# ZhangXinWhut/SimWhisper-Codec

Hardware: AMD Instinct MI355X
Metric: audio-sec/sec encode+decode (RTF^-1), 16kHz batch=32x10s (higher is better)
Workload: dtype split-f16 x3 encode (f32-class, f32 accumulate) / bf16 decode (f32 accumulate); 1 GPU; batch=32x10s @16kHz per GPU (32 utterances in all), encode()+decode(), 0.1*N(0,1) seed 1234, synthetic closed-form checkpoint (291M params); precision=mixed

## Files before the change

### include/swc.h

```cpp
#ifndef SWC_H_
#define SWC_H_

#include <stdint.h>

#ifdef __cplusplus
extern "C" {
#endif

#define SWC_OK 0
#define SWC_E_ARG (-1)
#define SWC_E_LAUNCH (-2)
#define SWC_E_NODEV (-3)

#define SWC_F32 0
#define SWC_BF16 1
#define SWC_F16S 2
#define SWC_F16S_ACT_SCALE 64.0f
#define SWC_FP8 3
#define SWC_FP8_ACT_SCALE 16.0f
#define SWC_F16 4

#define SWC_ACT_NONE 0
#define SWC_ACT_GELU 1

int swc_version(void);
const char* swc_last_error(void);
int swc_device_count(void);

int swc_delay_us(int32_t us, void* stream);

int swc_set_saturation_counter(uint32_t* counters);

typedef struct swc_gemm_args {
    const void* A;
    const void* W;
    void* C;
    const float* bias;
    const float* gamma;
    const float* residual;
    int64_t lda, ldw, ldc, ldr;
    int32_t M, N, K;
    int32_t taps, dil, stride, pad, t_in, t_out;
    int32_t a_dtype, c_dtype, act;
    float alpha;
    float out_scale;
} swc_gemm_args;
int swc_gemm(const swc_gemm_args* args, void* stream);

int swc_attention(const void* qkv, void* out, const int32_t* lens, int32_t B, int32_t T,
                  int32_t H, int32_t dtype, void* stream);
int swc_attention16(const void* qkv, void* out, const int32_t* lens, int32_t B, int32_t T, int32_t H,
                    int32_t dtype, const int32_t* row_start, void* stream);
int swc_attention_ex(const void* qkv, void* out, const int32_t* lens, int32_t B, int32_t T, int32_t H,
                     int32_t out_dtype, void* stream);

int swc_layernorm(const float* x, void* y, const float* w, const float* b, const int32_t* lens,
                  int32_t B, int32_t t_in, int32_t t_out, int32_t C, float eps, int32_t y_dtype,
                  const int32_t* row_start, void* stream);

int swc_pack_rows(const void* src, void* dst, const int32_t* row_start, const int32_t* lens, int32_t B, int32_t T,
                  int64_t row_bytes, void* stream);

int64_t swc_convnext_stream_bytes(int32_t C, int32_t I);
int swc_convnext_pack(const void* w1_16bit, const void* w2_16bit, const float* gamma, void* w_stream, int32_t C, int32_t I,
                      void* stream);
int swc_convnext_mlp(const void* y, const void* w_stream, const float* b1, const float* b2, const float* gamma,
                     float* x, int32_t M, int32_t C, int32_t I, void* stream);
int swc_convnext_block(const float* x, float* x_out, const float* dw_w7, const float* dw_bias, const float* ln_w,
                       const float* ln_b, float eps, const void* w_stream, const float* b1, const float* b2,
                       const float* gamma, int32_t B, int32_t T, int32_t C, int32_t I, const int32_t* t_limit,
                       int32_t operand_dtype, void* stream);

int64_t swc_convnext64_stream_bytes(int32_t C, int32_t I);
int swc_convnext64_pack(const void* w1_bf16, const void* w2_bf16, void* w_stream, int32_t C, int32_t I, void* stream);
int swc_convnext64_mlp(const void* y, const void* w_stream, const float* b1, const float* b2, const float* gamma, float* x,
                       int32_t M, int32_t C, int32_t I, int32_t stagger_cycles, void* stream);

int64_t swc_mlp_stream_bytes(int32_t D, int32_t F);
int swc_mlp_pack(const void* w1_bf16, const void* w2_bf16, void* w_stream, int32_t D, int32_t F, void* stream);
int swc_mlp_block(const float* x, float* x_out, const float* ln_w, const float* ln_b, float eps, const void* w_stream,
                  const float* b1, const float* b2, const float* next_ln_w, const float* next_ln_b, void* y_next,
                  int32_t M, int32_t D, int32_t F, void* stream);

int64_t swc_layer_tail_stream_bytes(int32_t D, int32_t F, int32_t fc1_dtype);
int swc_layer_tail_pack(const void* wo_bf16, const void* w1, const void* w2_bf16, void* w_stream, int32_t D, int32_t F,
                        int32_t fc1_dtype, void* stream);
int swc_layer_tail(const void* attn, const float* x, float* x_out, const void* w_stream, const float* bo, const float* ln_w,
                   const float* ln_b, float eps, const float* b1, const float* b2, const float* next_ln_w,
                   const float* next_ln_b, void* y_next, int32_t M, int32_t D, int32_t F, int32_t fc1_dtype, float fc1_alpha,
                   int32_t operand_dtype, void* stream);

int64_t swc_proj_ln_stream_bytes(int32_t N, int32_t K);
int swc_proj_ln_pack(const void* w_f16s, void* w_stream, int32_t N, int32_t K, void* stream);
int swc_proj_ln(const void* a_f16s, int64_t lda, const void* w_stream, const float* bias, float alpha, const float* x,
                float* x_out, const float* ln_w, const float* ln_b, float eps, void* y_next, int32_t M, int32_t N, int32_t K,
                void* stream);

int swc_dwconv7_ln(const float* x, void* y, const float* w, const float* bias, const float* ln_w,
                   const float* ln_b, int32_t B, int32_t T, int32_t C, float eps, int32_t y_dtype,
                   void* stream);

int swc_snake_aa(const float* x, void* y, const float* alpha, const float* beta,
                 const float* filt_host12, int32_t B, int32_t T, int32_t C, int32_t y_dtype,
                 void* stream);

int swc_fsq_encode(const float* z, int64_t ldz, float* zq, int32_t* codes, const int32_t* lens,
                   const float* consts_host12, int32_t B, int32_t T, int32_t t_pad, int32_t G,
                   void* stream);
int swc_fsq_decode(const int64_t* codes, float* zq, int64_t ldq, const int32_t* lens, int32_t B,
                   int32_t T, int32_t G, void* stream);
int swc_fsq_encode_levels(const float* z, int64_t ldz, float* zq, int32_t* codes, const int32_t* lens,
                          const float* consts_host12, const int32_t* levels_host4, int32_t B, int32_t T,
                          int32_t t_pad, int32_t G, void* stream);
int swc_fsq_decode_levels(const int64_t* codes, float* zq, int64_t ldq, const int32_t* lens,
                          const int32_t* levels_host4, int32_t B, int32_t T, int32_t G, void* stream);

int swc_mel_frames(const float* wav, int64_t ld_wav, const int32_t* n, int32_t n_pad,
                   float* frames, int32_t B, int32_t T, void* stream);
int swc_mel_power(const float* dft, int64_t ld, float* pw, int64_t ldp, int64_t rows,
                  void* stream);
int swc_mel_logmax(float* mel, int64_t ld, float* umax, int32_t B, int32_t T, int32_t n_mel,
                   void* stream);
int swc_mel_final(const float* mel, int64_t ld, const float* umax, void* out, int64_t ldo,
                  int32_t B, int32_t T, int32_t n_mel, int32_t out_dtype, void* stream);

int swc_deconv_col2im(const float* y3, const float* bias, void* out, int64_t ldo, int32_t B,
                      int32_t T, int32_t C, int32_t s, int32_t t_out, int32_t out_dtype,
                      void* stream);

int swc_istft_spec(const float* h, int64_t ldh, void* s, int64_t lds, int64_t rows,
                   int32_t s_dtype, void* stream);
int swc_istft_ola(const float* frames, const float* window_sq, float* wav, int32_t B, int32_t T,
                  void* stream);

int swc_codes_pack(const int32_t* codes, int64_t ldg, void* bytes, int32_t T, void* stream);
int swc_codes_unpack(const void* bytes, int32_t* codes, int64_t ldg, int32_t T, void* stream);

int swc_cast_f32_bf16(const float* x, void* y, int64_t n, void* stream);
int swc_cast_f32_f16s(const float* x, int64_t ldx, void* y, int64_t rows, int32_t K, float scale,
                      void* stream);
int swc_cast_fp8(const void* x, int32_t x_dtype, void* y, int64_t n, float scale, void* stream);

int swc_gather_rows(const void* const* src, const int64_t* nbytes, void* out, int64_t ld_bytes, int32_t n_rows,
                    void* stream);

int swc_pcm16_to_f32(const int16_t* pcm, float* out, int64_t n, void* stream);
int swc_f32_to_pcm16(const float* x, int16_t* pcm, int64_t n, void* stream);


#ifdef __cplusplus
}
#endif
#endif
```

### simwhisper_codec_amd/_lib.py

```python
import ctypes as C
import os

import torch

HERE = os.path.dirname(os.path.abspath(__file__))
LIB_PATH = os.environ.get("SWC_LIB") or os.path.join(HERE, "libswc_hip.so")

F32, BF16, F16S, FP8 = 0, 1, 2, 3
F16S_ACT_SCALE = 64.0
FP8_ACT_SCALE = 16.0
ACT_NONE, ACT_GELU = 0, 1


class SwcError(RuntimeError):
    pass


class GemmArgs(C.Structure):
    _fields_ = [
        ("A", C.c_void_p), ("W", C.c_void_p), ("C", C.c_void_p),
        ("bias", C.c_void_p), ("gamma", C.c_void_p), ("residual", C.c_void_p),
        ("lda", C.c_int64), ("ldw", C.c_int64), ("ldc", C.c_int64), ("ldr", C.c_int64),
        ("M", C.c_int32), ("N", C.c_int32), ("K", C.c_int32),
        ("taps", C.c_int32), ("dil", C.c_int32), ("stride", C.c_int32), ("pad", C.c_int32),
        ("t_in", C.c_int32), ("t_out", C.c_int32),
        ("a_dtype", C.c_int32), ("c_dtype", C.c_int32), ("act", C.c_int32),
        ("alpha", C.c_float), ("out_scale", C.c_float),
    ]


_P, _I, _L, _F = C.c_void_p, C.c_int32, C.c_int64, C.c_float

SIGNATURES = {
    "swc_gemm": [C.POINTER(GemmArgs), _P],
    "swc_attention": [_P, _P, _P, _I, _I, _I, _I, _P],
    "swc_attention_ex": [_P, _P, _P, _I, _I, _I, _I, _P],
    "swc_attention16": [_P, _P, _P, _I, _I, _I, _I, _P, _P],
    "swc_layernorm": [_P, _P, _P, _P, _P, _I, _I, _I, _I, _F, _I, _P, _P],
    "swc_dwconv7_ln": [_P, _P, _P, _P, _P, _P, _I, _I, _I, _F, _I, _P],
    "swc_snake_aa": [_P, _P, _P, _P, C.POINTER(_F), _I, _I, _I, _I, _P],
    "swc_fsq_encode": [_P, _L, _P, _P, _P, C.POINTER(_F), _I, _I, _I, _I, _P],
    "swc_fsq_decode": [_P, _P, _L, _P, _I, _I, _I, _P],
    "swc_fsq_encode_levels": [_P, _L, _P, _P, _P, C.POINTER(_F), C.POINTER(C.c_int32), _I, _I, _I, _I, _P],
    "swc_fsq_decode_levels": [_P, _P, _L, _P, C.POINTER(C.c_int32), _I, _I, _I, _P],
    "swc_mel_frames": [_P, _L, _P, _I, _P, _I, _I, _P],
    "swc_mel_power": [_P, _L, _P, _L, _L, _P],
    "swc_mel_logmax": [_P, _L, _P, _I, _I, _I, _P],
    "swc_mel_final": [_P, _L, _P, _P, _L, _I, _I, _I, _I, _P],
    "swc_deconv_col2im": [_P, _P, _P, _L, _I, _I, _I, _I, _I, _I, _P],
    "swc_istft_spec": [_P, _L, _P, _L, _L, _I, _P],
    "swc_istft_ola": [_P, _P, _P, _I, _I, _P],
    "swc_codes_pack": [_P, _L, _P, _I, _P],
    "swc_codes_unpack": [_P, _P, _L, _I, _P],
    "swc_cast_f32_bf16": [_P, _P, _L, _P],
    "swc_cast_f32_f16s": [_P, _L, _P, _L, _I, _F, _P],
    "swc_cast_fp8": [_P, _I, _P, _L, _F, _P],
    "swc_gather_rows": [_P, _P, _P, _L, _I, _P],
    "swc_pcm16_to_f32": [_P, _P, _L, _P],
    "swc_f32_to_pcm16": [_P, _P, _L, _P],
    "swc_set_saturation_counter": [_P],
    "swc_delay_us": [_I, _P],
    "swc_pack_rows": [_P, _P, _P, _P, _I, _I, _L, _P],
    "swc_convnext_pack": [_P, _P, _P, _P, _I, _I, _P],
    "swc_convnext_mlp": [_P, _P, _P, _P, _P, _P, _I, _I, _I, _P],
    "swc_convnext_block": [_P, _P, _P, _P, _P, _P, _F, _P, _P, _P, _P, _I, _I, _I, _I, _P, _I, _P],
    "swc_convnext64_pack": [_P, _P, _P, _I, _I, _P],
    "swc_convnext64_mlp": [_P, _P, _P, _P, _P, _P, _I, _I, _I, _I, _P],
    "swc_mlp_pack": [_P, _P, _P, _I, _I, _P],
    "swc_mlp_block": [_P, _P, _P, _P, _F, _P, _P, _P, _P, _P, _P, _I, _I, _I, _P],
    "swc_layer_tail_pack": [_P, _P, _P, _P, _I, _I, _I, _P],
    "swc_layer_tail": [_P, _P, _P, _P, _P, _P, _P, _F, _P, _P, _P, _P, _P, _I, _I, _I, _I, _F, _I, _P],
    "swc_proj_ln_pack": [_P, _P, _I, _I, _P],
    "swc_proj_ln": [_P, _L, _P, _P, _F, _P, _P, _P, _P, _F, _P, _I, _I, _I, _P],
}
PLAIN = {"swc_version": ([], C.c_int), "swc_last_error": ([], C.c_char_p), "swc_device_count": ([], C.c_int),
         "swc_convnext_stream_bytes": ([_I, _I], C.c_int64),
         "swc_mlp_stream_bytes": ([_I, _I], C.c_int64), "swc_convnext64_stream_bytes": ([_I, _I], C.c_int64), "swc_layer_tail_stream_bytes": ([_I, _I, _I], C.c_int64),
         "swc_proj_ln_stream_bytes": ([_I, _I], C.c_int64)}

_lib = None


def load():
    global _lib
    if _lib is not None:
        return _lib
    if not os.path.exists(LIB_PATH):
        raise SwcError(
            f"{LIB_PATH} is missing: build it with `python -m simwhisper_codec_amd.build` "
            "(there is no CPU or PyTorch fallback for the hot path)")
    lib = C.CDLL(LIB_PATH)
    for name, argtypes in SIGNATURES.items():
        fn = getattr(lib, name)
        fn.argtypes = argtypes
        fn.restype = C.c_int
    for name, (argtypes, restype) in PLAIN.items():
        fn = getattr(lib, name)
        fn.argtypes = argtypes
        fn.restype = restype
    _lib = lib
    return lib


def check(rc, what):
    if rc != 0:
        msg = load().swc_last_error().decode("utf-8", "replace")
        raise SwcError(f"{what} failed (rc={rc}): {msg}")


def exported_symbols():
    return list(SIGNATURES) + list(PLAIN)
```

### simwhisper_codec_amd/csrc/swc_attention16.hip

```cpp
#include "swc_common.h"
#include <type_traits>

namespace {

typedef short s16x4 __attribute__((ext_vector_type(4)));
typedef short s16x8 __attribute__((ext_vector_type(8)));

__device__ __attribute__((aligned(16))) unsigned int g_zero16a[4] = {0u, 0u, 0u, 0u};

__device__ __forceinline__ void glds16a(const void* gsrc, unsigned lds_addr) {
    unsigned keep;
    asm volatile(
        "s_mov_b32 %0, m0\n\ts_mov_b32 m0, %2\n\ts_nop 0\n\tglobal_load_lds_dwordx4 %1, off\n\ts_mov_b32 m0, %0"
        : "=&s"(keep)
        : "v"(gsrc), "s"(lds_addr)
        : "memory");
}

typedef unsigned u32x2_sw __attribute__((ext_vector_type(2)));
template <int W>
__device__ __forceinline__ float xor_max(float v) {
    const unsigned u = __float_as_uint(v);
    const u32x2_sw r = W == 16 ? __builtin_amdgcn_permlane16_swap(u, u, false, false) : __builtin_amdgcn_permlane32_swap(u, u, false, false);
    return fmaxf(__uint_as_float(r[0]), __uint_as_float(r[1]));
}

template <int PLANES>
__device__ __forceinline__ f32x4 mma16(const uint4& a, const uint4& b, f32x4 c) {
#if defined(ATT_ABL) && (ATT_ABL & 8)
    c[0] += __uint_as_float(a.x ^ b.x);
    return c;
#endif
    if constexpr (PLANES == 1)
        return __builtin_amdgcn_mfma_f32_16x16x32_bf16(*reinterpret_cast<const bf16x8*>(&a),
                                                       *reinterpret_cast<const bf16x8*>(&b), c, 0, 0, 0);
    else
        return __builtin_amdgcn_mfma_f32_16x16x32_f16(*reinterpret_cast<const f16x8*>(&a),
                                                      *reinterpret_cast<const f16x8*>(&b), c, 0, 0, 0);
}

typedef float f32x2 __attribute__((ext_vector_type(2)));
typedef __bf16 bf16x2n __attribute__((ext_vector_type(2)));
typedef _Float16 f16x2 __attribute__((ext_vector_type(2)));
__device__ __forceinline__ unsigned pack2_bf16(float lo, float hi) {
    const bf16x2n r = __builtin_convertvector((f32x2){lo, hi}, bf16x2n);
    return *reinterpret_cast<const unsigned*>(&r);
}
__device__ __forceinline__ unsigned pack2_f16(float lo, float hi) {
    const f16x2 r = __builtin_convertvector((f32x2){lo, hi}, f16x2);
    return *reinterpret_cast<const unsigned*>(&r);
}


template <int PLANES, int KT16, int NQT, bool RES = false>
__global__ __launch_bounds__(RES ? 512 : 256, RES ? 1 : (NQT == 1 ? 4 : 2)) void attn16_kernel(const char* __restrict__ qkv, unsigned short* __restrict__ out,
                                                        const int* __restrict__ lens, int T, int H,
                                                        const int* __restrict__ row_start) {
    constexpr int ROWB = 128 * PLANES;
    constexpr int CPR = ROWB / 16;
    constexpr int TILE = KT16 * ROWB;
    constexpr int QB16 = 64 * NQT;
    constexpr int QW = 16 * NQT;
    constexpr int NKS = KT16 / 16;
    constexpr int NPR = KT16 / 32;
    constexpr int NI = TILE / 1024;
    extern __shared__ __attribute__((aligned(16))) char smem[];

    constexpr int NW = RES ? 8 : 4;
    const int b = blockIdx.z, head = blockIdx.y;
    int q0 = RES ? 0 : blockIdx.x * QB16;
    const int tid = threadIdx.x, lane = tid & 63, wave = tid >> 6;
    const int fr = lane & 15, fh = lane >> 4;
    const int D = H * 64;
    const long ldb = 3L * D * 2 * PLANES;
    const long part = (long)D * 2 * PLANES;
    int len = lens[b];
    len = len < 0 ? 0 : (len > T ? T : len);
    const long r0 = row_start ? (long)row_start[b] : (long)b * T;
    const int qlim = row_start ? len : T;
    const char* base = qkv + r0 * ldb + (long)head * ROWB;

    auto krow_swz = [](int row) { return PLANES == 1 ? (((row >> 1) ^ ((row >> 4) << 1)) & 7) : (row & 15); };
    auto vrow_swz = [](int row) { return PLANES == 1 ? ((row >> 1) & 3) : (row & 7); };

    auto store_o = [&](int q, int d, float a, float bq, float c, float e) {
        if (q >= qlim) return;
        if constexpr (PLANES == 1) {
            uint2 u;
            u.x = bf16_pack2(a, bq);
            u.y = bf16_pack2(c, e);
            *reinterpret_cast<uint2*>(out + (r0 + q) * D + head * 64 + d) = u;
        } else {
            f16s_store4(out + (r0 + q) * 2L * D, head * 64 + d, a, bq, c, e);
        }
    };

    if (!RES && q0 >= len) {
#pragma unroll
        for (int qt = 0; qt < NQT; ++qt)
#pragma unroll
            for (int dt = 0; dt < 4; ++dt) store_o(q0 + wave * QW + qt * 16 + fr, dt * 16 + fh * 4, 0.f, 0.f, 0.f, 0.f);
        return;
    }

    uint4 qf[NQT][2][PLANES];
    auto load_q = [&]() {
#pragma unroll
        for (int qt = 0; qt < NQT; ++qt) {
            int q = q0 + wave * QW + qt * 16 + fr;
            q = q < qlim ? q : qlim - 1;
            const char* qp = base + (long)q * ldb;
#pragma unroll
            for (int g = 0; g < 2; ++g)
#pragma unroll
                for (int pl = 0; pl < PLANES; ++pl) {
                    const int c = PLANES == 1 ? (4 * g + fh) : (8 * g + 4 * pl + fh);
                    qf[qt][g][pl] = *reinterpret_cast<const uint4*>(qp + 16 * c);
                }
        }
    };

    const unsigned smem_base = __builtin_amdgcn_readfirstlane((unsigned)(uintptr_t)(const __attribute__((address_space(3))) char*)smem);
    const int wave_u = __builtin_amdgcn_readfirstlane(wave);
    const int l_row = lane / CPR, l_pos = lane % CPR;
    auto stage = [&](int kt, int st) {
        const int k0 = kt * KT16;
        const char* zero = reinterpret_cast<const char*>(g_zero16a);
#pragma unroll
        for (int j = 0; j < (NI + NW - 1) / NW; ++j) {
            const int inst = wave_u + NW * j;
            if (NI % NW != 0 && inst >= NI) break;
            const int row = inst * (64 / CPR) + l_row;
            const int key = k0 + row;
            const bool ok = key < len;
            const char* rp = base + (long)(ok ? key : 0) * ldb;
            const int kc = l_pos ^ krow_swz(row);
            const int vu = (l_pos >> 1) ^ vrow_swz(row);
            const char* ks = rp + part + 16 * kc;
            const char* vs = rp + 2 * part + 16 * ((vu << 1) | (l_pos & 1));
            glds16a(ok ? ks : zero, smem_base + st * 2 * TILE + inst * 1024);
            glds16a(ok ? vs : zero, smem_base + st * 2 * TILE + TILE + inst * 1024);
        }
    };
    auto fence = [&]() {
#if defined(ATT_ABL) && (ATT_ABL & 1)
        asm volatile("s_waitcnt vmcnt(0)" ::: "memory");
#elif defined(ATT_ABL) && (ATT_ABL & 2)
#else
        asm volatile("s_waitcnt vmcnt(0)" ::: "memory");
        __syncthreads();
#endif
    };

    f32x4 o[NQT][4];
    float m_run[NQT];
    f32x4 lacc[NQT];
    auto init_acc = [&]() {
#pragma unroll
        for (int qt = 0; qt < NQT; ++qt) {
#pragma unroll
            for (int dt = 0; dt < 4; ++dt) o[qt][dt] = (f32x4){0.f, 0.f, 0.f, 0.f};
            m_run[qt] = -INFINITY;
            lacc[qt] = (f32x4){0.f, 0.f, 0.f, 0.f};
        }
    };
    const unsigned one2 = PLANES == 1 ? 0x3F803F80u : 0x3C003C00u;
    const uint4 ones = make_uint4(one2, one2, one2, one2);
    const float c_exp = (PLANES == 1 ? 1.0f : 1.0f / (SWC_F16S_ACT_SCALE * SWC_F16S_ACT_SCALE)) * 1.4426950408889634f;
    const float m_off = PLANES == 1 ? 0.0f : 11.0f / c_exp;

    const int ntile = (len + KT16 - 1) / KT16;
    auto tile = [&](int kt, auto last_c) {
        constexpr bool LAST = decltype(last_c)::value;
        const int st = RES ? kt : (kt & 1);
#if !(defined(ATT_ABL) && (ATT_ABL & 32))
        if (!RES && !LAST) stage(kt + 1, st ^ 1);
#endif
        const char* sK = smem + st * 2 * TILE;
        const char* sV = sK + TILE;
        const int k0 = kt * KT16;

        f32x4 s[NQT][NKS];
#pragma unroll
        for (int ks = 0; ks < NKS; ++ks) {
            const int row = ks * 16 + fr;
            uint4 kf[2][PLANES];
#pragma unroll
            for (int g = 0; g < 2; ++g)
#pragma unroll
                for (int pl = 0; pl < PLANES; ++pl) {
                    const int c = PLANES == 1 ? (4 * g + fh) : (8 * g + 4 * pl + fh);
#if defined(ATT_ABL) && (ATT_ABL & 16)
                    kf[g][pl] = qf[0][g][pl];
#else
                    kf[g][pl] = *reinterpret_cast<const uint4*>(sK + row * ROWB + ((c ^ krow_swz(row)) << 4));
#endif
                }
#pragma unroll
            for (int qt = 0; qt < NQT; ++qt) {
                f32x4 a = (f32x4){0.f, 0.f, 0.f, 0.f};
#pragma unroll
                for (int g = 0; g < 2; ++g) {
                    if constexpr (PLANES == 2) {
                        a = mma16<PLANES>(kf[g][1], qf[qt][g][0], a);
                        a = mma16<PLANES>(kf[g][0], qf[qt][g][1], a);
                    }
                    a = mma16<PLANES>(kf[g][0], qf[qt][g][0], a);
                }
                s[qt][ks] = a;
            }
        }
        uint4 pf[NQT][NPR][PLANES];
#if defined(ATT_ABL) && (ATT_ABL & 4)
#pragma unroll
        for (int qt = 0; qt < NQT; ++qt)
#pragma unroll
            for (int pr = 0; pr < NPR; ++pr)
#pragma unroll
                for (int pl = 0; pl < PLANES; ++pl)
                    pf[qt][pr][pl] = *reinterpret_cast<uint4*>(&s[qt][(2 * pr + pl) % NKS]);
#else
#pragma unroll
        for (int qt = 0; qt < NQT; ++qt) {
            float mt = -INFINITY;
#pragma unroll
            for (int ks = 0; ks < NKS; ++ks)
#pragma unroll
                for (int e = 0; e < 4; ++e) {
                    const int key = k0 + ks * 16 + fh * 4 + e;
                    float v = s[qt][ks][e];
                    if (LAST) v = key < len ? v : -INFINITY;
                    s[qt][ks][e] = v;
                    mt = fmaxf(mt, v);
                }
            if constexpr (PLANES == 1) {
                mt = xor_max<16>(mt);
                mt = xor_max<32>(mt);
            } else {
                mt = fmaxf(mt, __shfl_xor(mt, 16));
                mt = fmaxf(mt, __shfl_xor(mt, 32));
            }
            bool rescale = true;
            if constexpr (PLANES == 1) rescale = __builtin_amdgcn_ballot_w64(mt > m_run[qt] + 8.0f / c_exp) != 0;
            float alpha = 1.0f;
            if (rescale) {
                const float m_new = fmaxf(m_run[qt], mt);
                alpha = __builtin_amdgcn_exp2f((m_run[qt] - m_new) * c_exp);
                m_run[qt] = m_new;
            }
            const float m_sub = m_run[qt] - m_off;
            const float mc = m_sub * c_exp;
            (void)mc;
#pragma unroll
            for (int ks = 0; ks < NKS; ++ks)
#pragma unroll
                for (int e = 0; e < 4; ++e) {
                    s[qt][ks][e] = PLANES == 1 ? __builtin_amdgcn_exp2f(fmaf(s[qt][ks][e], c_exp, -mc))
                                               : __builtin_amdgcn_exp2f((s[qt][ks][e] - m_sub) * c_exp);
                }
            if (rescale) {
                lacc[qt] *= alpha;
#pragma unroll
                for (int dt = 0; dt < 4; ++dt) o[qt][dt] *= alpha;
            }
#pragma unroll
            for (int pr = 0; pr < NPR; ++pr) {
                unsigned h[4], lo[4];
                (void)lo;
#pragma unroll
                for (int j2 = 0; j2 < 4; ++j2) {
                    const float p0 = s[qt][2 * pr + (j2 >> 1)][2 * (j2 & 1)], p1 = s[qt][2 * pr + (j2 >> 1)][2 * (j2 & 1) + 1];
                    if constexpr (PLANES == 1) {
                        h[j2] = pack2_bf16(p0, p1);
                    } else {
                        h[j2] = pack2_f16(p0, p1);
                        const f16x2 hh = *reinterpret_cast<const f16x2*>(&h[j2]);
                        lo[j2] = pack2_f16(p0 - (float)hh[0], p1 - (float)hh[1]);
                    }
                }
                pf[qt][pr][0] = make_uint4(h[0], h[1], h[2], h[3]);
                if constexpr (PLANES == 2) pf[qt][pr][1] = make_uint4(lo[0], lo[1], lo[2], lo[3]);
            }
        }
#endif
        const int tq = fr >> 2, tp = fr & 3;
#pragma unroll
        for (int pr = 0; pr < NPR; ++pr)
#pragma unroll
            for (int dt = 0; dt < 4; ++dt) {
                uint4 vf[PLANES];
#pragma unroll
                for (int pl = 0; pl < PLANES; ++pl) {
                    const int u = PLANES == 1 ? dt : ((dt >> 1) * 4 + (dt & 1) + 2 * pl);
                    s16x4 part2[2];
#pragma unroll
                    for (int t = 0; t < 2; ++t) {
                        const int row = (2 * pr + t) * 16 + 4 * fh + tq;
                        const char* ap = sV + row * ROWB + ((u ^ vrow_swz(row)) << 5) + 8 * tp;
                        part2[t] = __builtin_amdgcn_ds_read_tr16_b64_v4i16(
                            (__attribute__((address_space(3))) s16x4*)(uintptr_t)(unsigned)(uintptr_t)(const __attribute__((address_space(3))) char*)ap);
                    }
                    s16x8 full = __builtin_shufflevector(part2[0], part2[1], 0, 1, 2, 3, 4, 5, 6, 7);
                    vf[pl] = *reinterpret_cast<uint4*>(&full);
#if defined(ATT_ABL) && (ATT_ABL & 16)
                    vf[pl] = qf[0][pl & 1][0];
#endif
                }
#pragma unroll
                for (int qt = 0; qt < NQT; ++qt) {
                    f32x4 a = o[qt][dt];
                    if constexpr (PLANES == 2) {
                        a = mma16<PLANES>(vf[1], pf[qt][pr][0], a);
                        a = mma16<PLANES>(vf[0], pf[qt][pr][1], a);
                    }
                    a = mma16<PLANES>(vf[0], pf[qt][pr][0], a);
                    o[qt][dt] = a;
                }
            }
#pragma unroll
        for (int pr = 0; pr < NPR; ++pr)
#pragma unroll
            for (int qt = 0; qt < NQT; ++qt) {
                if constexpr (PLANES == 2) lacc[qt] = mma16<PLANES>(ones, pf[qt][pr][1], lacc[qt]);
                lacc[qt] = mma16<PLANES>(ones, pf[qt][pr][0], lacc[qt]);
            }
        if (!RES) fence();
    };
    auto finish = [&]() {
#pragma unroll
        for (int qt = 0; qt < NQT; ++qt) {
            const float l = lacc[qt][0];
            const float inv = l > 0.f ? 1.0f / l : 0.f;
            const int q = q0 + wave * QW + qt * 16 + fr;
#pragma unroll
            for (int dt = 0; dt < 4; ++dt) {
                const f32x4 v = o[qt][dt] * inv;
                store_o(q, dt * 16 + fh * 4, v[0], v[1], v[2], v[3]);
            }
        }
    };
    if constexpr (RES) {
        for (int kt = 0; kt < ntile; ++kt) stage(kt, kt);
        fence();
        for (q0 = 0; q0 < qlim; q0 += NW * QW) {
            if (q0 + wave * QW >= len || ntile == 0) {
#pragma unroll
                for (int qt = 0; qt < NQT; ++qt)
#pragma unroll
                    for (int dt = 0; dt < 4; ++dt) store_o(q0 + wave * QW + qt * 16 + fr, dt * 16 + fh * 4, 0.f, 0.f, 0.f, 0.f);
                continue;
            }
            load_q();
            init_acc();
            for (int kt = 0; kt + 1 < ntile; ++kt) tile(kt, std::false_type{});
            tile(ntile - 1, std::true_type{});
            finish();
        }
    } else {
        load_q();
        init_acc();
        stage(0, 0);
        fence();
        for (int kt = 0; kt + 1 < ntile; ++kt) tile(kt, std::false_type{});
        tile(ntile - 1, std::true_type{});
        finish();
    }
}

#ifndef ATT_RES
#define ATT_RES 0
#endif
int launch16_resident(const void* qkv, void* out, const int32_t* lens, int B, int T, int H, const int32_t* row_start, hipStream_t s) {
    constexpr int LDS = 8 * 2 * 64 * 128;
    auto kern = attn16_kernel<1, 64, 2, true>;
    SWC_ENABLE_LDS(kern, LDS, "swc_attention16");
    dim3 grid(1, H, B), block(512);
    hipLaunchKernelGGL(kern, grid, block, LDS, s, (const char*)qkv, (unsigned short*)out, lens, T, H, row_start);
    return SWC_OK;
}

template <int PLANES, int KT16, int NQT>
int launch16(const void* qkv, void* out, const int32_t* lens, int B, int T, int H, const int32_t* row_start, hipStream_t s) {
    constexpr int LDS = 2 * 2 * KT16 * 128 * PLANES;
    auto kern = attn16_kernel<PLANES, KT16, NQT>;
    constexpr int QB16 = 64 * NQT;
    if (LDS > 48 * 1024) SWC_ENABLE_LDS(kern, LDS, "swc_attention16");
    dim3 grid((T + QB16 - 1) / QB16, H, B), block(256);
    hipLaunchKernelGGL(kern, grid, block, LDS, s, (const char*)qkv, (unsigned short*)out, lens, T, H, row_start);
    return SWC_OK;
}

}

extern "C" int swc_attention16(const void* qkv, void* out, const int32_t* lens, int32_t B, int32_t T, int32_t H,
                               int32_t dtype, const int32_t* row_start, void* stream) {
    SWC_CHECK_ARG(qkv && out && lens, "swc_attention16: null pointer");
    SWC_CHECK_ARG(B >= 0 && T >= 0 && H > 0 && B <= 65535 && H <= 65535, "swc_attention16: bad B/T/H");
    SWC_CHECK_ARG(dtype == SWC_BF16 || dtype == SWC_F16S, "swc_attention16: dtype must be BF16 or F16S");
    SWC_CHECK_ARG(aligned16(qkv) && aligned16(out), "swc_attention16: unaligned");
    if (B == 0 || T == 0) return SWC_OK;
    int rc = dtype == SWC_BF16 ? ((ATT_RES && T <= 512) ? launch16_resident(qkv, out, lens, B, T, H, row_start, (hipStream_t)stream)
                                                        : launch16<1, 64, 2>(qkv, out, lens, B, T, H, row_start, (hipStream_t)stream))
                               : launch16<2, 64, 2>(qkv, out, lens, B, T, H, row_start, (hipStream_t)stream);
    if (rc != SWC_OK) return rc;
    SWC_CHECK_LAUNCH("swc_attention16");
    return SWC_OK;
}
```

Baseline: 15070 audio-s/s.

## Remap attention16 grid to XCD-aware flat walk over batch-head-qblock items

The 3D attention grid becomes a 1D grid. Each workgroup walks work items (batch, head, query block) strided so that items sharing a batch-head land on the same XCD, which should improve L2 reuse of K/V. The code also adds optional persistent-grid and next-item prefetch variants behind ATT_WALK, plus higher occupancy bounds for the bf16 walk path. Because ATT_WALK defaults to 1, only the XCD remap with a full-size grid runs by default; the old grid path stays available as swc_attention16_grid.

```diff
diff --git a/include/swc.h b/include/swc.h
--- a/include/swc.h
+++ b/include/swc.h
@@ -51,6 +51,8 @@
                   int32_t H, int32_t dtype, void* stream);
 int swc_attention16(const void* qkv, void* out, const int32_t* lens, int32_t B, int32_t T, int32_t H,
                     int32_t dtype, const int32_t* row_start, void* stream);
+int swc_attention16_grid(const void* qkv, void* out, const int32_t* lens, int32_t B, int32_t T, int32_t H,
+                         int32_t dtype, const int32_t* row_start, void* stream);
 int swc_attention_ex(const void* qkv, void* out, const int32_t* lens, int32_t B, int32_t T, int32_t H,
                      int32_t out_dtype, void* stream);
 
diff --git a/simwhisper_codec_amd/_lib.py b/simwhisper_codec_amd/_lib.py
--- a/simwhisper_codec_amd/_lib.py
+++ b/simwhisper_codec_amd/_lib.py
@@ -36,6 +36,7 @@
     "swc_attention": [_P, _P, _P, _I, _I, _I, _I, _P],
     "swc_attention_ex": [_P, _P, _P, _I, _I, _I, _I, _P],
     "swc_attention16": [_P, _P, _P, _I, _I, _I, _I, _P, _P],
+    "swc_attention16_grid": [_P, _P, _P, _I, _I, _I, _I, _P, _P],
     "swc_layernorm": [_P, _P, _P, _P, _P, _I, _I, _I, _I, _F, _I, _P, _P],
     "swc_dwconv7_ln": [_P, _P, _P, _P, _P, _P, _I, _I, _I, _F, _I, _P],
     "swc_snake_aa": [_P, _P, _P, _P, C.POINTER(_F), _I, _I, _I, _I, _P],
diff --git a/simwhisper_codec_amd/csrc/swc_attention16.hip b/simwhisper_codec_amd/csrc/swc_attention16.hip
--- a/simwhisper_codec_amd/csrc/swc_attention16.hip
+++ b/simwhisper_codec_amd/csrc/swc_attention16.hip
@@ -52,9 +52,9 @@
 }
 
 
-template <int PLANES, int KT16, int NQT, bool RES = false>
-__global__ __launch_bounds__(RES ? 512 : 256, RES ? 1 : (NQT == 1 ? 4 : 2)) void attn16_kernel(const char* __restrict__ qkv, unsigned short* __restrict__ out,
-                                                        const int* __restrict__ lens, int T, int H,
+template <int PLANES, int KT16, int NQT, bool RES = false, int WALK = 0>
+__global__ __launch_bounds__(RES ? 512 : 256, RES ? 1 : ((NQT == 1 || (WALK && PLANES == 1)) ? 4 : 2)) void attn16_kernel(const char* __restrict__ qkv, unsigned short* __restrict__ out,
+                                                        const int* __restrict__ lens, int B, int T, int H,
                                                         const int* __restrict__ row_start) {
     constexpr int ROWB = 128 * PLANES;
     constexpr int CPR = ROWB / 16;
@@ -67,49 +67,66 @@
     extern __shared__ __attribute__((aligned(16))) char smem[];
 
     constexpr int NW = RES ? 8 : 4;
-    const int b = blockIdx.z, head = blockIdx.y;
-    int q0 = RES ? 0 : blockIdx.x * QB16;
     const int tid = threadIdx.x, lane = tid & 63, wave = tid >> 6;
     const int fr = lane & 15, fh = lane >> 4;
     const int D = H * 64;
     const long ldb = 3L * D * 2 * PLANES;
     const long part = (long)D * 2 * PLANES;
-    int len = lens[b];
-    len = len < 0 ? 0 : (len > T ? T : len);
-    const long r0 = row_start ? (long)row_start[b] : (long)b * T;
-    const int qlim = row_start ? len : T;
-    const char* base = qkv + r0 * ldb + (long)head * ROWB;
+
+    struct Item {
+        int head, q0, len, qlim;
+        long r0;
+        const char* base;
+    };
+    auto make_item = [&](int b, int head, int q0) {
+        Item it;
+        it.head = head;
+        it.q0 = q0;
+        int len = lens[b];
+        it.len = len < 0 ? 0 : (len > T ? T : len);
+        it.r0 = row_start ? (long)row_start[b] : (long)b * T;
+        it.qlim = row_start ? it.len : T;
+        it.base = qkv + it.r0 * ldb + (long)head * ROWB;
+        return it;
+    };
+    Item cur = RES ? make_item(blockIdx.z, blockIdx.y, 0) : make_item(WALK ? 0 : blockIdx.z, WALK ? 0 : blockIdx.y, WALK ? 0 : blockIdx.x * QB16);
+    Item nxt = cur;
+    bool has_next = false;
+    int sb = 0;
 
     auto krow_swz = [](int row) { return PLANES == 1 ? (((row >> 1) ^ ((row >> 4) << 1)) & 7) : (row & 15); };
     auto vrow_swz = [](int row) { return PLANES == 1 ? ((row >> 1) & 3) : (row & 7); };
 
-    auto store_o = [&](int q, int d, float a, float bq, float c, float e) {
-        if (q >= qlim) return;
+    auto store_o = [&](const Item& it, int q, int d, float a, float bq, float c, float e) {
+        if (q >= it.qlim) return;
         if constexpr (PLANES == 1) {
             uint2 u;
             u.x = bf16_pack2(a, bq);
             u.y = bf16_pack2(c, e);
-            *reinterpret_cast<uint2*>(out + (r0 + q) * D + head * 64 + d) = u;
+            *reinterpret_cast<uint2*>(out + (it.r0 + q) * D + it.head * 64 + d) = u;
         } else {
-            f16s_store4(out + (r0 + q) * 2L * D, head * 64 + d, a, bq, c, e);
-        }
-    };
-
-    if (!RES && q0 >= len) {
+            f16s_store4(out + (it.r0 + q) * 2L * D, it.head * 64 + d, a, bq, c, e);
+        }
+    };
+    auto zero_fill = [&](const Item& it) {
 #pragma unroll
         for (int qt = 0; qt < NQT; ++qt)
 #pragma unroll
-            for (int dt = 0; dt < 4; ++dt) store_o(q0 + wave * QW + qt * 16 + fr, dt * 16 + fh * 4, 0.f, 0.f, 0.f, 0.f);
+            for (int dt = 0; dt < 4; ++dt) store_o(it, it.q0 + wave * QW + qt * 16 + fr, dt * 16 + fh * 4, 0.f, 0.f, 0.f, 0.f);
+    };
+
+    if (!RES && !WALK && cur.q0 >= cur.len) {
+        zero_fill(cur);
         return;
     }
 
     uint4 qf[NQT][2][PLANES];
-    auto load_q = [&]() {
+    auto load_q = [&](const Item& it) {
 #pragma unroll
         for (int qt = 0; qt < NQT; ++qt) {
-            int q = q0 + wave * QW + qt * 16 + fr;
-            q = q < qlim ? q : qlim - 1;
-            const char* qp = base + (long)q * ldb;
+            int q = it.q0 + wave * QW + qt * 16 + fr;
+            q = q < it.qlim ? q : it.qlim - 1;
+            const char* qp = it.base + (long)q * ldb;
 #pragma unroll
             for (int g = 0; g < 2; ++g)
 #pragma unroll
@@ -123,7 +140,7 @@
     const unsigned smem_base = __builtin_amdgcn_readfirstlane((unsigned)(uintptr_t)(const __attribute__((address_space(3))) char*)smem);
     const int wave_u = __builtin_amdgcn_readfirstlane(wave);
     const int l_row = lane / CPR, l_pos = lane % CPR;
-    auto stage = [&](int kt, int st) {
+    auto stage = [&](const Item& it, int kt, int st) {
         const int k0 = kt * KT16;
         const char* zero = reinterpret_cast<const char*>(g_zero16a);
 #pragma unroll
@@ -132,8 +149,8 @@
             if (NI % NW != 0 && inst >= NI) break;
             const int row = inst * (64 / CPR) + l_row;
             const int key = k0 + row;
-            const bool ok = key < len;
-            const char* rp = base + (long)(ok ? key : 0) * ldb;
+            const bool ok = key < it.len;
+            const char* rp = it.base + (long)(ok ? key : 0) * ldb;
             const int kc = l_pos ^ krow_swz(row);
             const int vu = (l_pos >> 1) ^ vrow_swz(row);
             const char* ks = rp + part + 16 * kc;
@@ -169,12 +186,13 @@
     const float c_exp = (PLANES == 1 ? 1.0f : 1.0f / (SWC_F16S_ACT_SCALE * SWC_F16S_ACT_SCALE)) * 1.4426950408889634f;
     const float m_off = PLANES == 1 ? 0.0f : 11.0f / c_exp;
 
-    const int ntile = (len + KT16 - 1) / KT16;
     auto tile = [&](int kt, auto last_c) {
         constexpr bool LAST = decltype(last_c)::value;
-        const int st = RES ? kt : (kt & 1);
+        const int len = cur.len;
+        const int st = RES ? kt : ((kt + sb) & 1);
 #if !(defined(ATT_ABL) && (ATT_ABL & 32))
-        if (!RES && !LAST) stage(kt + 1, st ^ 1);
+        if (!RES && !LAST) stage(cur, kt + 1, st ^ 1);
+        if (WALK == 2 && LAST && has_next) stage(nxt, 0, st ^ 1);
 #endif
         const char* sK = smem + st * 2 * TILE;
         const char* sV = sK + TILE;
@@ -331,39 +349,77 @@
         for (int qt = 0; qt < NQT; ++qt) {
             const float l = lacc[qt][0];
             const float inv = l > 0.f ? 1.0f / l : 0.f;
-            const int q = q0 + wave * QW + qt * 16 + fr;
+            const int q = cur.q0 + wave * QW + qt * 16 + fr;
 #pragma unroll
             for (int dt = 0; dt < 4; ++dt) {
                 const f32x4 v = o[qt][dt] * inv;
-                store_o(q, dt * 16 + fh * 4, v[0], v[1], v[2], v[3]);
+                store_o(cur, q, dt * 16 + fh * 4, v[0], v[1], v[2], v[3]);
             }
         }
     };
     if constexpr (RES) {
-        for (int kt = 0; kt < ntile; ++kt) stage(kt, kt);
+        const int ntile = (cur.len + KT16 - 1) / KT16;
+        for (int kt = 0; kt < ntile; ++kt) stage(cur, kt, kt);
         fence();
-        for (q0 = 0; q0 < qlim; q0 += NW * QW) {
-            if (q0 + wave * QW >= len || ntile == 0) {
-#pragma unroll
-                for (int qt = 0; qt < NQT; ++qt)
-#pragma unroll
-                    for (int dt = 0; dt < 4; ++dt) store_o(q0 + wave * QW + qt * 16 + fr, dt * 16 + fh * 4, 0.f, 0.f, 0.f, 0.f);
+        for (cur.q0 = 0; cur.q0 < cur.qlim; cur.q0 += NW * QW) {
+            if (cur.q0 + wave * QW >= cur.len || ntile == 0) {
+                zero_fill(cur);
                 continue;
             }
-            load_q();
+            load_q(cur);
             init_acc();
             for (int kt = 0; kt + 1 < ntile; ++kt) tile(kt, std::false_type{});
             tile(ntile - 1, std::true_type{});
             finish();
         }
-    } else {
-        load_q();
+    } else if constexpr (WALK == 0) {
+        const int ntile = (cur.len + KT16 - 1) / KT16;
+        load_q(cur);
         init_acc();
-        stage(0, 0);
+        stage(cur, 0, 0);
         fence();
         for (int kt = 0; kt + 1 < ntile; ++kt) tile(kt, std::false_type{});
         tile(ntile - 1, std::true_type{});
         finish();
+    } else {
+        const int nqb = (T + QB16 - 1) / QB16;
+        const int xcd = blockIdx.x & 7;
+        const int gw = ((int)gridDim.x - xcd + 7) >> 3;
+        const int nloc = ((B * H - xcd + 7) >> 3) * nqb;
+        auto seek = [&](int& l, Item& it) {
+            for (; l < nloc; l += gw) {
+                const int pl = l / nqb, p = xcd + 8 * pl, b = p / H;
+                it = make_item(b, p - b * H, (l - pl * nqb) * QB16);
+                if (it.q0 < it.len) return true;
+                if (!row_start) zero_fill(it);
+            }
+            return false;
+        };
+        int l = blockIdx.x >> 3;
+        if (!seek(l, cur)) return;
+        load_q(cur);
+        init_acc();
+        stage(cur, 0, 0);
+        fence();
+        for (;;) {
+            const int ntile = (cur.len + KT16 - 1) / KT16;
+            int ln = l + gw;
+            has_next = seek(ln, nxt);
+            for (int kt = 0; kt + 1 < ntile; ++kt) tile(kt, std::false_type{});
+            tile(ntile - 1, std::true_type{});
+            if (WALK == 2 && has_next) load_q(nxt);
+            finish();
+            if (!has_next) break;
+            sb = (sb + ntile) & 1;
+            cur = nxt;
+            l = ln;
+            if (WALK != 2) load_q(cur);
+            init_acc();
+            if (WALK != 2) {
+                stage(cur, 0, sb);
+                fence();
+            }
+        }
     }
 }
 
@@ -375,34 +431,85 @@
     auto kern = attn16_kernel<1, 64, 2, true>;
     SWC_ENABLE_LDS(kern, LDS, "swc_attention16");
     dim3 grid(1, H, B), block(512);
-    hipLaunchKernelGGL(kern, grid, block, LDS, s, (const char*)qkv, (unsigned short*)out, lens, T, H, row_start);
+    hipLaunchKernelGGL(kern, grid, block, LDS, s, (const char*)qkv, (unsigned short*)out, lens, B, T, H, row_start);
     return SWC_OK;
 }
 
-template <int PLANES, int KT16, int NQT>
+#ifndef ATT_WALK
+#define ATT_WALK 1
+#endif
+
+template <typename K>
+int resident_workgroups(K kern, int lds, int* n) {
+    static int cache[64] = {};
+    int dev = 0;
+    (void)hipGetDevice(&dev);
+    const int slot = (dev >= 0 && dev < 64) ? dev : 0;
+    if (cache[slot] == 0 || dev >= 64) {
+        int per_cu = 0, cus = 0;
+        hipError_t e = hipOccupancyMaxActiveBlocksPerMultiprocessor(&per_cu, reinterpret_cast<const void*>(kern), 256, lds);
+        if (e == hipSuccess) e = hipDeviceGetAttribute(&cus, hipDeviceAttributeMultiprocessorCount, dev);
+        if (e != hipSuccess || per_cu < 1 || cus < 1) {
+            swc_set_error("swc_attention16: occupancy query failed: %s", hipGetErrorString(e));
+            return SWC_E_LAUNCH;
+        }
+        cache[slot] = per_cu * cus;
+    }
+    *n = cache[slot];
+    return SWC_OK;
+}
+
+template <int PLANES, int KT16, int NQT, bool WALK>
 int launch16(const void* qkv, void* out, const int32_t* lens, int B, int T, int H, const int32_t* row_start, hipStream_t s) {
     constexpr int LDS = 2 * 2 * KT16 * 128 * PLANES;
-    auto kern = attn16_kernel<PLANES, KT16, NQT>;
     constexpr int QB16 = 64 * NQT;
-    if (LDS > 48 * 1024) SWC_ENABLE_LDS(kern, LDS, "swc_attention16");
-    dim3 grid((T + QB16 - 1) / QB16, H, B), block(256);
-    hipLaunchKernelGGL(kern, grid, block, LDS, s, (const char*)qkv, (unsigned short*)out, lens, T, H, row_start);
+    const int nqb = (T + QB16 - 1) / QB16;
+    if constexpr (!WALK) {
+        auto kern = attn16_kernel<PLANES, KT16, NQT, false, 0>;
+        if (LDS > 48 * 1024) SWC_ENABLE_LDS(kern, LDS, "swc_attention16");
+        dim3 grid(nqb, H, B), block(256);
+        hipLaunchKernelGGL(kern, grid, block, LDS, s, (const char*)qkv, (unsigned short*)out, lens, B, T, H, row_start);
+    } else {
+        auto kern = attn16_kernel<PLANES, KT16, NQT, false, ATT_WALK == 3 ? 2 : 1>;
+        if (LDS > 48 * 1024) SWC_ENABLE_LDS(kern, LDS, "swc_attention16");
+        const long items8 = 8L * (((long)B * H + 7) / 8) * nqb;
+        SWC_CHECK_ARG(items8 <= 0x7fffffffL, "swc_attention16: too many work items");
+        long grid = items8;
+        if (ATT_WALK >= 2) {
+            int res = 0;
+            const int rc = resident_workgroups(kern, LDS, &res);
+            if (rc != SWC_OK) return rc;
+            grid = grid < res ? grid : res;
+        }
+        hipLaunchKernelGGL(kern, dim3((unsigned)grid), dim3(256), LDS, s, (const char*)qkv, (unsigned short*)out, lens, B, T, H, row_start);
+    }
     return SWC_OK;
 }
 
-}
-
-extern "C" int swc_attention16(const void* qkv, void* out, const int32_t* lens, int32_t B, int32_t T, int32_t H,
-                               int32_t dtype, const int32_t* row_start, void* stream) {
+template <bool WALK>
+int attention16(const void* qkv, void* out, const int32_t* lens, int32_t B, int32_t T, int32_t H, int32_t dtype,
+                const int32_t* row_start, void* stream) {
     SWC_CHECK_ARG(qkv && out && lens, "swc_attention16: null pointer");
     SWC_CHECK_ARG(B >= 0 && T >= 0 && H > 0 && B <= 65535 && H <= 65535, "swc_attention16: bad B/T/H");
     SWC_CHECK_ARG(dtype == SWC_BF16 || dtype == SWC_F16S, "swc_attention16: dtype must be BF16 or F16S");
     SWC_CHECK_ARG(aligned16(qkv) && aligned16(out), "swc_attention16: unaligned");
     if (B == 0 || T == 0) return SWC_OK;
     int rc = dtype == SWC_BF16 ? ((ATT_RES && T <= 512) ? launch16_resident(qkv, out, lens, B, T, H, row_start, (hipStream_t)stream)
-                                                        : launch16<1, 64, 2>(qkv, out, lens, B, T, H, row_start, (hipStream_t)stream))
-                               : launch16<2, 64, 2>(qkv, out, lens, B, T, H, row_start, (hipStream_t)stream);
+                                                        : launch16<1, 64, 2, WALK>(qkv, out, lens, B, T, H, row_start, (hipStream_t)stream))
+                               : launch16<2, 64, 2, WALK>(qkv, out, lens, B, T, H, row_start, (hipStream_t)stream);
     if (rc != SWC_OK) return rc;
     SWC_CHECK_LAUNCH("swc_attention16");
     return SWC_OK;
 }
+
+}
+
+extern "C" int swc_attention16(const void* qkv, void* out, const int32_t* lens, int32_t B, int32_t T, int32_t H,
+                               int32_t dtype, const int32_t* row_start, void* stream) {
+    return attention16<ATT_WALK != 0>(qkv, out, lens, B, T, H, dtype, row_start, stream);
+}
+
+extern "C" int swc_attention16_grid(const void* qkv, void* out, const int32_t* lens, int32_t B, int32_t T, int32_t H,
+                                    int32_t dtype, const int32_t* row_start, void* stream) {
+    return attention16<false>(qkv, out, lens, B, T, H, dtype, row_start, stream);
+}
```

New measurement: 15140 audio-s/s, median of 6. Within noise of the previous version (+0.4%).
